# vaenyr/stable-diffusion-on-device

Measured on AMD Instinct MI355X. Metric: images/sec + per-UNet-step ms, SD v1.4 512x512 20-step PLMS, 1/2/4/8 MI355X, higher is better.
Workload: dtype f16

## Files before the change

### stable-diffusion-on-device_amd/csrc/attention.hip

```cpp
#include "common.h"
#include "sdod_hip.h"
#include "host_util.h"

#include <cstdlib>
#include <type_traits>

namespace {

struct AttnP {
    const f16* q;
    const f16* k;
    const f16* v;
    f16* out;
    int B, H, Lq, Lk;
    int ldq, ldk, ldv, ldo;
    float scale_log2;
    int causal;
};

typedef short short4v __attribute__((__vector_size__(4 * sizeof(short))));
typedef __attribute__((address_space(3))) short4v* lds_short4_ptr;

constexpr int odd16(int dv) {
    int s = (dv + 15) / 16;
    if ((s & 1) == 0) s += 1;
    return s * 16;
}

template <int D, int QT>
constexpr int attn_min_waves() { return (D == 40 || (D == 80 && QT == 1)) ? 3 : 1; }

template <int N, int I = 0, class F>
SDOD_DEVICE void static_for(F&& f) {
    if constexpr (I < N) {
        f(std::integral_constant<int, I>{});
        static_for<N, I + 1>(f);
    }
}

template <int D, int QT, bool TR, int KVS = 1>
__global__ __launch_bounds__(256 * KVS, (attn_min_waves<D, QT>())) void attn_kernel(const AttnP p) {
    constexpr int DP = ((D + 31) / 32) * 32;
    constexpr int KSTEPS = DP / 32;
    constexpr int DV = ((D + 15) / 16) * 16;
    constexpr int NDT = DV / 16;
    constexpr int KSTR = DP + 8;
    constexpr int VSTR = odd16(DV);
    constexpr int KT = 64;
    constexpr int DC = D / 8;
    constexpr int LD_IT = (KT * DC + 255) / 256;
    constexpr int STAGE = KT * (KSTR + VSTR);
    constexpr bool SUM_BY_MFMA = DV > D;
    static_assert(D % 8 == 0, "head dim must be a multiple of 8");

    extern __shared__ __attribute__((aligned(16))) char smem_raw[];
    const int grp = KVS > 1 ? (int)(threadIdx.x >> 8) : 0;
    f16* smem = reinterpret_cast<f16*>(smem_raw) + (size_t)grp * 2 * STAGE;

    const int tid = threadIdx.x & 255;
    const int lane = tid & 63;
    const int wave = tid >> 6;
    const int g = lane >> 4;
    const int li = lane & 15;
    const int nqb = (p.Lq + 64 * QT - 1) / (64 * QT);
    const int lid = xcd_remap(blockIdx.x, nqb * p.H * p.B);
    const int bh = lid / nqb;
    const int b = bh / p.H, h = bh - b * p.H;
    const int q_block = (lid - bh * nqb) * (64 * QT);

    const f16* kbase = p.k + (size_t)b * p.Lk * p.ldk + h * D;
    const f16* vbase = p.v + (size_t)b * p.Lk * p.ldv + h * D;

    {
        constexpr int KPADC = (DP - D) / 8, VPADC = (DV - D) / 8;
        for (int st = 0; st < 2; ++st) {
            f16* sK = smem + st * STAGE;
            f16* sV = sK + KT * KSTR;
            if (KPADC > 0)
                for (int idx = tid; idx < KT * KPADC; idx += 256) {
                    const int row = idx / (KPADC > 0 ? KPADC : 1), ch = idx - row * KPADC;
                    *reinterpret_cast<f16x8*>(sK + row * KSTR + D + ch * 8) = zero8();
                }
            if (VPADC > 0)
                for (int idx = tid; idx < KT * VPADC; idx += 256) {
                    const int row = idx / (VPADC > 0 ? VPADC : 1), ch = idx - row * VPADC;
                    f16x8 pad = zero8();
                    if (ch == 0) pad[0] = (f16)1.0f;
                    *reinterpret_cast<f16x8*>(sV + row * VSTR + D + ch * 8) = pad;
                }
        }
    }

    f16x8 qf[QT][KSTEPS];
    int qrow[QT];
#pragma unroll
    for (int t = 0; t < QT; ++t) {
        qrow[t] = q_block + wave * (16 * QT) + t * 16 + li;
        const f16* qp = p.q + ((size_t)b * p.Lq + qrow[t]) * p.ldq + h * D;
#pragma unroll
        for (int ks = 0; ks < KSTEPS; ++ks) {
            const int d0 = ks * 32 + g * 8;
            qf[t][ks] = (qrow[t] < p.Lq && d0 + 8 <= D) ? ldg8(qp + d0) : zero8();
        }
    }

    int kend = p.Lk;
    if (p.causal) kend = min(p.Lk, q_block + 64 * QT);
    const int NT = (kend + KT - 1) / KT;

    f16x8 rk[LD_IT], rv[LD_IT];
    const f16* kptr0[LD_IT];
    const f16* vptr0[LD_IT];
#pragma unroll
    for (int i = 0; i < LD_IT; ++i) {
        const int idx = tid + 256 * i;
        const int row = idx / DC, ch = idx - row * DC;
        kptr0[i] = kbase + (size_t)row * p.ldk + ch * 8;
        vptr0[i] = vbase + (size_t)row * p.ldv + ch * 8;
    }
    auto load_tile = [&](int t) {
        if (t * KT + KT <= p.Lk) {
            const size_t ko = (size_t)t * KT * p.ldk, vo = (size_t)t * KT * p.ldv;
#pragma unroll
            for (int i = 0; i < LD_IT; ++i) {
                if (tid + 256 * i < KT * DC) {
                    rk[i] = ldg8(kptr0[i] + ko);
                    rv[i] = ldg8(vptr0[i] + vo);
                }
            }
            return;
        }
#pragma unroll
        for (int i = 0; i < LD_IT; ++i) {
            const int idx = tid + 256 * i;
            const int row = idx / DC, ch = idx - row * DC;
            const int key = t * KT + row;
            const bool ok = (idx < KT * DC) && (key < p.Lk);
            rk[i] = ok ? ldg8(kbase + (size_t)key * p.ldk + ch * 8) : zero8();
            rv[i] = ok ? ldg8(vbase + (size_t)key * p.ldv + ch * 8) : zero8();
        }
    };
    auto store_tile = [&](int st) {
        f16* sK = smem + st * STAGE;
        f16* sV = sK + KT * KSTR;
#pragma unroll
        for (int i = 0; i < LD_IT; ++i) {
            const int idx = tid + 256 * i;
            const int row = idx / DC, ch = idx - row * DC;
            if (idx < KT * DC) {
                *reinterpret_cast<f16x8*>(sK + row * KSTR + ch * 8) = rk[i];
                *reinterpret_cast<f16x8*>(sV + row * VSTR + ch * 8) = rv[i];
            }
        }
    };

    f32x4 o[QT][NDT];
    float m_run[QT], l_run[QT];
#pragma unroll
    for (int t = 0; t < QT; ++t) {
        m_run[t] = -1e30f;
        l_run[t] = 0.f;
#pragma unroll
        for (int dt = 0; dt < NDT; ++dt) o[t][dt] = f32x4{0.f, 0.f, 0.f, 0.f};
    }

#ifdef SDOD_ATTN_ABLATE
    constexpr int abl = SDOD_ATTN_ABLATE;
#else
    constexpr int abl = 0;
#endif
    constexpr bool HOLD = D <= 80;
    auto read_vt = [&](const f16* sV, int u, int dt) -> f16x8 {
        const f16* a0 = sV + (32 * u + 4 * g + (li >> 2)) * VSTR + dt * 16 + 4 * (li & 3);
        const short4v lo = __builtin_amdgcn_ds_read_tr16_b64_v4i16((lds_short4_ptr)(a0));
        const short4v hi = __builtin_amdgcn_ds_read_tr16_b64_v4i16((lds_short4_ptr)(a0 + 16 * VSTR));
        typedef short short8v __attribute__((__vector_size__(8 * sizeof(short))));
        const short8v both = __builtin_shufflevector(lo, hi, 0, 1, 2, 3, 4, 5, 6, 7);
        return __builtin_bit_cast(f16x8, both);
    };
    auto softmax_pv = [&](auto a_c, int t, f32x4 (&s_a)[4], const f16x8 (&vfr)[HOLD ? 2 : 1][HOLD ? NDT : 1], const f16* sV) {
        constexpr int a = decltype(a_c)::value;
        const bool need_mask = (t * KT + KT > p.Lk) || (p.causal && (t * KT + KT - 1 > q_block + wave * (16 * QT)));
        if (need_mask) {
            int key0 = t * KT + g * 4;
            asm volatile("" : "+v"(key0));
#pragma unroll
            for (int c = 0; c < 4; ++c)
#pragma unroll
                for (int r = 0; r < 4; ++r) {
                    const int key = key0 + c * 16 + r;
                    const bool masked = (key >= p.Lk) | (p.causal & (key > qrow[a]));
                    s_a[c][r] = masked ? -1e30f : s_a[c][r];
                }
        }
        float mx;
        {
            const float t0 = fmaxf(fmaxf(s_a[0][0], s_a[0][1]), s_a[0][2]);
            const float t1 = fmaxf(fmaxf(s_a[0][3], s_a[1][0]), s_a[1][1]);
            const float t2 = fmaxf(fmaxf(s_a[1][2], s_a[1][3]), s_a[2][0]);
            const float t3 = fmaxf(fmaxf(s_a[2][1], s_a[2][2]), s_a[2][3]);
            const float t4 = fmaxf(fmaxf(s_a[3][0], s_a[3][1]), s_a[3][2]);
            const float u0 = fmaxf(fmaxf(t0, t1), t2);
            const float u1 = fmaxf(fmaxf(t3, t4), s_a[3][3]);
            mx = fmaxf(u0, u1);
        }
        mx = quad_rows_max(mx);
        const float m_new = fmaxf(m_run[a], mx * p.scale_log2);
        const bool rescale = __builtin_amdgcn_ballot_w64(m_new != m_run[a]) != 0;
        const float alpha = rescale ? __builtin_amdgcn_exp2f(m_run[a] - m_new) : 1.0f;
        m_run[a] = m_new;
        float rs[4] = {0.f, 0.f, 0.f, 0.f};
        const float sc = p.scale_log2, nm = -m_new;
#pragma unroll
        for (int c = 0; c < 4; ++c) {
#pragma unroll
            for (int r = 0; r < 4; ++r) {
                float v = __builtin_fmaf(s_a[c][r], sc, nm);
                if (!(abl & 2)) v = __builtin_amdgcn_exp2f(v);
                if (!SUM_BY_MFMA) rs[r] += v;
                s_a[c][r] = v;
            }
        }
        if (!SUM_BY_MFMA) l_run[a] = __builtin_fmaf(l_run[a], alpha, (rs[0] + rs[1]) + (rs[2] + rs[3]));
        if (rescale) {
#pragma unroll
            for (int dt = 0; dt < NDT; ++dt)
#pragma unroll
                for (int r = 0; r < 4; ++r) o[a][dt][r] *= alpha;
        }
        f16x8 pf[2];
#pragma unroll
        for (int u = 0; u < 2; ++u) {
            f16x8 f;
#pragma unroll
            for (int r = 0; r < 4; ++r) {
                f[r] = (f16)s_a[2 * u][r];
                f[4 + r] = (f16)s_a[2 * u + 1][r];
            }
            pf[u] = f;
        }
#pragma unroll
        for (int u = 0; u < 2; ++u) {
#pragma unroll
            for (int dt = 0; dt < NDT; ++dt) {
                f16x8 vf;
                if (TR) {
                    vf = HOLD ? vfr[u][dt] : read_vt(sV, u, dt);
                } else {
#pragma unroll
                    for (int e = 0; e < 8; ++e) vf[e] = sV[(32 * u + 16 * (e >> 2) + 4 * g + (e & 3)) * VSTR + dt * 16 + li];
                }
                o[a][dt] = mfma16(vf, pf[u], o[a][dt]);
            }
        }
    };
    auto read_k = [&](const f16* sK, f16x8 (&kf)[HOLD ? KSTEPS : 1][4]) {
        if constexpr (HOLD) {
#pragma unroll
            for (int ks = 0; ks < KSTEPS; ++ks)
#pragma unroll
                for (int c = 0; c < 4; ++c) kf[ks][c] = *reinterpret_cast<const f16x8*>(sK + (c * 16 + li) * KSTR + ks * 32 + g * 8);
        }
    };
    auto read_v = [&](const f16* sV, f16x8 (&vfr)[HOLD ? 2 : 1][HOLD ? NDT : 1]) {
        if constexpr (TR && HOLD) {
#pragma unroll
            for (int u = 0; u < 2; ++u)
#pragma unroll
                for (int dt = 0; dt < NDT; ++dt) vfr[u][dt] = read_vt(sV, u, dt);
        }
    };
    auto qk = [&](const f16* sK, const f16x8 (&kf)[HOLD ? KSTEPS : 1][4], f32x4 (&s)[QT][4]) {
#pragma unroll
        for (int a = 0; a < QT; ++a) {
#pragma unroll
            for (int c = 0; c < 4; ++c) s[a][c] = f32x4{0.f, 0.f, 0.f, 0.f};
#pragma unroll
            for (int ks = 0; ks < KSTEPS; ++ks)
#pragma unroll
                for (int c = 0; c < 4; ++c) {
                    const f16x8 k8 = HOLD ? kf[ks][c] : *reinterpret_cast<const f16x8*>(sK + (c * 16 + li) * KSTR + ks * 32 + g * 8);
                    s[a][c] = mfma16(k8, qf[a][ks], s[a][c]);
                }
        }
    };

    if (grp < NT) {
        load_tile(grp);
        store_tile(0);
    }
    __syncthreads();
    const int NTG = (NT + KVS - 1) / KVS;
    for (int it = 0; it < NTG; ++it) {
        const int t = it * KVS + grp;
        const int cur = it & 1;
        const bool has_next = t + KVS < NT;
        const f16* sK = smem + cur * STAGE;
        const f16* sV = sK + KT * KSTR;
        if (t >= NT) {
            __syncthreads();
            continue;
        }
        f16x8 kf[HOLD ? KSTEPS : 1][4];
        f16x8 vfr[HOLD ? 2 : 1][HOLD ? NDT : 1];
        read_k(sK, kf);
        read_v(sV, vfr);
        f32x4 s[QT][4];
        qk(sK, kf, s);
        if (has_next && !(abl & 1)) load_tile(t + KVS);
        static_for<QT>([&](auto a_c) { softmax_pv(a_c, t, s[decltype(a_c)::value], vfr, sV); });
        if (has_next) store_tile(cur ^ 1);
        __syncthreads();
    }

    if constexpr (KVS > 1) {
        static_assert(KVS == 2, "the merge below handles two groups");
        float* mrg = reinterpret_cast<float*>(smem_raw);
        constexpr int NV = QT * (2 + NDT * 4);
        static_assert((size_t)NV * 256 * sizeof(float) <= (size_t)KVS * 2 * STAGE * sizeof(f16), "merge buffer fits the staging LDS");
        if (grp == 1) {
#pragma unroll
            for (int a = 0; a < QT; ++a) {
                mrg[(a * (2 + NDT * 4) + 0) * 256 + tid] = m_run[a];
                mrg[(a * (2 + NDT * 4) + 1) * 256 + tid] = l_run[a];
#pragma unroll
                for (int dt = 0; dt < NDT; ++dt)
#pragma unroll
                    for (int r = 0; r < 4; ++r) mrg[(a * (2 + NDT * 4) + 2 + dt * 4 + r) * 256 + tid] = o[a][dt][r];
            }
        }
        __syncthreads();
        if (grp == 1) return;
#pragma unroll
        for (int a = 0; a < QT; ++a) {
            const float m1 = mrg[(a * (2 + NDT * 4) + 0) * 256 + tid], l1 = mrg[(a * (2 + NDT * 4) + 1) * 256 + tid];
            const float m = fmaxf(m_run[a], m1);
            const float a0 = __builtin_amdgcn_exp2f(m_run[a] - m), a1 = __builtin_amdgcn_exp2f(m1 - m);
            l_run[a] = l_run[a] * a0 + l1 * a1;
#pragma unroll
            for (int dt = 0; dt < NDT; ++dt)
#pragma unroll
                for (int r = 0; r < 4; ++r) o[a][dt][r] = o[a][dt][r] * a0 + mrg[(a * (2 + NDT * 4) + 2 + dt * 4 + r) * 256 + tid] * a1;
            m_run[a] = m;
        }
    }
#pragma unroll
    for (int a = 0; a < QT; ++a) {
        float l;
        if (SUM_BY_MFMA) {
            l = __shfl(o[a][D / 16][D % 4], ((D % 16) / 4) * 16 + li);
        } else {
            l = quad_rows_sum(l_run[a]);
        }
        const float inv = l > 0.f ? 1.0f / l : 0.f;
        if (qrow[a] < p.Lq) {
            f16* op = p.out + ((size_t)b * p.Lq + qrow[a]) * p.ldo + h * D;
#pragma unroll
            for (int dt = 0; dt < NDT; ++dt) {
                const int dv0 = dt * 16 + g * 4;
                if (dv0 < D) {
                    f16x4 hv;
#pragma unroll
                    for (int r = 0; r < 4; ++r) hv[r] = (f16)(o[a][dt][r] * inv);
                    *reinterpret_cast<f16x4*>(op + dv0) = hv;
                }
            }
        }
    }
}

template <int D, int QT, bool TR, int KVS = 1>
hipError_t attn_launch(const AttnP& p, hipStream_t st) {
    constexpr int DP = ((D + 31) / 32) * 32;
    constexpr int DV = ((D + 15) / 16) * 16;
    constexpr size_t smem = (size_t)KVS * 2 * 64 * (DP + 8 + odd16(DV)) * sizeof(f16);
    static_assert(smem <= 160 * 1024, "LDS");
    static std::atomic<unsigned long long> attr_devs{0};
    if (sdod::first_use_on_device(attr_devs)) {
        hipError_t e = hipFuncSetAttribute(reinterpret_cast<const void*>(&attn_kernel<D, QT, TR, KVS>),
                                           hipFuncAttributeMaxDynamicSharedMemorySize, (int)smem);
        if (e != hipSuccess) return e;
    }
    dim3 grid(((p.Lq + 64 * QT - 1) / (64 * QT)) * p.H * p.B);
    SDOD_LAUNCH((attn_kernel<D, QT, TR, KVS>), grid, dim3(256 * KVS), smem, st, p);
    return hipGetLastError();
}

template <int D>
hipError_t attn_dispatch(const AttnP& p, bool big, bool tr, hipStream_t st) {
    if (tr) return big ? attn_launch<D, 2, true>(p, st) : attn_launch<D, 1, true>(p, st);
    return big ? attn_launch<D, 2, false>(p, st) : attn_launch<D, 1, false>(p, st);
}

struct FoldP {
    const f16* kv; int ld_kv, k_off, v_off, L, n_img;
    const f16* wq; int ldq;
    const float* sq; const float* tq;
    const f16* wo; int ldwo;
    int heads, d, C;
    float alpha;
    f16* w1; float* s1; float* t1; f16* w2;
    int tiles_c;
    int n_w;
};
constexpr int kFoldKMax = 160;
__global__ __launch_bounds__(256) void xattn_fold_kernel(const FoldP p) {
    __shared__ __attribute__((aligned(16))) f16 sa[80][kFoldKMax + 8], sb[80][kFoldKMax + 8];
    const int tid = threadIdx.x, lane = tid & 63, wave = tid >> 6;
    const int NK = p.heads * 80, d = p.d;
    int item = blockIdx.x;
    if (item >= 2 * p.n_w) {
        const int idx = (item - 2 * p.n_w) * 256 + tid;
        if (idx >= p.n_img * NK) return;
        const int j = idx % 80, bh = idx / 80, h = bh % p.heads, img = bh / p.heads;
        if (j >= p.L) {
            p.s1[idx] = 0.f;
            p.t1[idx] = -30000.f;
            return;
        }
        const f16* kr = p.kv + ((long long)img * p.L + j) * p.ld_kv + p.k_off + h * d;
        float a = 0.f, b = 0.f;
        for (int dd = 0; dd < d; ++dd) {
            const float kval = (float)kr[dd];
            a = fmaf(kval, p.sq[h * d + dd], a);
            b = fmaf(kval, p.tq[h * d + dd], b);
        }
        p.s1[idx] = p.alpha * a;
        p.t1[idx] = p.alpha * b;
        return;
    }
    const bool second = item >= p.n_w;
    if (second) item -= p.n_w;
    const int tc = item % p.tiles_c, bh = item / p.tiles_c, h = bh % p.heads, img = bh / p.heads;
    const int KP = (d + 31) & ~31, kc = KP / 8;
    auto stage_rows = [&](f16 (*dst)[kFoldKMax + 8], const f16* base, long long row_stride, int valid_rows) {
        for (int idx = tid; idx < 80 * kc; idx += 256) {
            const int r = idx / kc, ch = idx - r * kc;
            const f16x8 v = (r < valid_rows && ch * 8 < d) ? ldg8(base + (long long)r * row_stride + ch * 8) : zero8();
            *reinterpret_cast<f16x8*>(&dst[r][ch * 8]) = v;
        }
    };
    if (!second) {
        stage_rows(sa, p.kv + (long long)img * p.L * p.ld_kv + p.k_off + h * d, p.ld_kv, p.L);
        for (int idx = tid; idx < KP * 10; idx += 256) {
            const int k = idx / 10, ch = idx - k * 10;
            const f16x8 v = k < d ? ldg8(p.wq + (long long)(h * d + k) * p.ldq + tc * 80 + ch * 8) : zero8();
#pragma unroll
            for (int e = 0; e < 8; ++e) sb[ch * 8 + e][k] = v[e];
        }
    } else {
        stage_rows(sa, p.wo + (long long)(tc * 80) * p.ldwo + h * d, p.ldwo, 80);
        stage_rows(sb, p.kv + (long long)img * p.L * p.ld_kv + p.v_off + h * d, p.ld_kv, p.L);
    }
    __syncthreads();
    const int fr = lane & 15, fg = lane >> 4;
    for (int rb = wave; rb < 5; rb += 4) {
        f32x4 acc[5];
#pragma unroll
        for (int j = 0; j < 5; ++j) acc[j] = f32x4{0.f, 0.f, 0.f, 0.f};
        for (int ks = 0; ks < KP / 32; ++ks) {
            const f16x8 fa = *reinterpret_cast<const f16x8*>(&sa[rb * 16 + fr][ks * 32 + fg * 8]);
#pragma unroll
            for (int j = 0; j < 5; ++j) {
                const f16x8 fb = *reinterpret_cast<const f16x8*>(&sb[j * 16 + fr][ks * 32 + fg * 8]);
                acc[j] = mfma16(fb, fa, acc[j]);
            }
        }
        const int m = rb * 16 + fr;
        f16* row = second ? p.w2 + ((long long)img * p.C + tc * 80 + m) * NK + h * 80
                          : p.w1 + ((long long)(img * p.heads + h) * 80 + m) * p.C + tc * 80;
        const float al = second ? 1.0f : p.alpha;
#pragma unroll
        for (int j = 0; j < 5; ++j) {
            f16x4 o;
#pragma unroll
            for (int r = 0; r < 4; ++r) o[r] = (f16)(al * acc[j][r]);
            *reinterpret_cast<f16x4*>(row + j * 16 + fg * 4) = o;
        }
    }
}

}

extern "C" int sdod_attention_f16(const void* q, const void* k, const void* v, void* out, int batch, int heads, int lq,
                                  int lk, int d, int ldq, int ldk, int ldv, int ldo, float scale, int causal,
                                  void* stream) {
    SDOD_TRY
    SDOD_REQUIRE(q && k && v && out, "null pointer");
    SDOD_REQUIRE(batch > 0 && heads > 0 && lq > 0 && lk > 0, "bad shape");
    SDOD_REQUIRE(d == 40 || d == 64 || d == 80 || d == 160, "head dim must be one of 40, 64, 80, 160");
    SDOD_REQUIRE(ldq % 8 == 0 && ldk % 8 == 0 && ldv % 8 == 0 && ldo % 4 == 0, "row strides must keep 16-byte alignment");
    SDOD_REQUIRE(ldq >= heads * d && ldk >= heads * d && ldv >= heads * d && ldo >= heads * d, "row stride < heads*d");
    SDOD_REQUIRE((((uintptr_t)q | (uintptr_t)k | (uintptr_t)v) & 15) == 0 && ((uintptr_t)out & 7) == 0, "misaligned pointer");
    AttnP p{};
    p.q = (const f16*)q; p.k = (const f16*)k; p.v = (const f16*)v; p.out = (f16*)out;
    p.B = batch; p.H = heads; p.Lq = lq; p.Lk = lk;
    p.ldq = ldq; p.ldk = ldk; p.ldv = ldv; p.ldo = ldo;
    p.scale_log2 = scale * 1.4426950408889634f;
    p.causal = causal;
    const bool no_tr = std::getenv("SDOD_ATTN_NO_TR") != nullptr;
    const bool tr = !no_tr;
    bool big = lq >= 2048 && d != 160;
    if (const char* e = std::getenv("SDOD_ATTN_QT")) big = e[0] == '2' && d != 160;
    hipStream_t st = (hipStream_t)stream;
    hipError_t e;
    switch (d) {
    case 40: e = attn_dispatch<40>(p, big, tr, st); break;
    case 64: e = attn_dispatch<64>(p, big, tr, st); break;
    case 80: {
        static const bool kvs_off = [] { const char* e2 = std::getenv("SDOD_ATTN_KVS"); return e2 && e2[0] == '0'; }();
        const long long wgs = (long long)((lq + 63) / 64) * heads * batch;
        if (!big && tr && !kvs_off && !causal && wgs <= 512 && lk >= 256) e = attn_launch<80, 1, true, 2>(p, st);
        else e = attn_dispatch<80>(p, big, tr, st);
        break;
    }
    default: e = attn_dispatch<160>(p, false, tr, st); break;
    }
    SDOD_HIP_CHECK(e);
    return 0;
    SDOD_CATCH
}

extern "C" int sdod_xattn_fold_f16(const void* kv, int ld_kv, int k_off, int v_off, int n_img, int L, const void* wq, int ldq,
                                   const void* sq, const void* tq, const void* wo, int ldwo, int heads, int d, float scale, void* w1,
                                   void* s1, void* t1, void* w2, void* stream) {
    SDOD_TRY
    SDOD_REQUIRE(kv && wq && sq && tq && wo && w1 && s1 && t1 && w2, "null pointer");
    SDOD_REQUIRE(n_img > 0 && heads > 0 && d > 0 && d <= kFoldKMax && d % 8 == 0 && L > 0 && L <= 80, "bad shape (d <= 160, d % 8 == 0, L <= 80)");
    const int C = heads * d, NK = heads * 80;
    SDOD_REQUIRE(C % 80 == 0 && ldq >= C && ldwo >= C && ld_kv >= C, "heads * d must be a multiple of 80; row strides >= heads * d");
    SDOD_REQUIRE(ld_kv % 8 == 0 && k_off % 8 == 0 && v_off % 8 == 0 && ldq % 8 == 0 && ldwo % 8 == 0 &&
                     (((uintptr_t)kv | (uintptr_t)wq | (uintptr_t)wo | (uintptr_t)w1 | (uintptr_t)w2) & 15) == 0,
                 "operands must keep 16-byte alignment");
    FoldP p{};
    p.kv = (const f16*)kv; p.ld_kv = ld_kv; p.k_off = k_off; p.v_off = v_off; p.L = L; p.n_img = n_img;
    p.wq = (const f16*)wq; p.ldq = ldq; p.sq = (const float*)sq; p.tq = (const float*)tq;
    p.wo = (const f16*)wo; p.ldwo = ldwo;
    p.heads = heads; p.d = d; p.C = C;
    p.alpha = scale * 1.4426950408889634f;
    p.w1 = (f16*)w1; p.s1 = (float*)s1; p.t1 = (float*)t1; p.w2 = (f16*)w2;
    p.tiles_c = C / 80;
    p.n_w = n_img * heads * p.tiles_c;
    const int blocks = 2 * p.n_w + (n_img * NK + 255) / 256;
    SDOD_LAUNCH(xattn_fold_kernel, dim3(blocks), dim3(256), 0, (hipStream_t)stream, p);
    SDOD_HIP_CHECK(hipGetLastError());
    return 0;
    SDOD_CATCH
}
```

Baseline: 10.47.

## Fold max subtraction into QK MFMA via padded K column and defer rescaling

For head dims with K padding (DP > D), Q is prescaled by scale*log2e and the running max is written into a padded Q lane, while the matching padded K column holds -1. The QK MFMA then emits scores already shifted by the running max. The online-softmax max and rescale of O and l are skipped unless some score exceeds a threshold (8 in log2 space), checked with an integer max and a wave ballot. This removes most per-tile fma and max-reduction work, but it quantises Q and the max to f16, which risks precision loss and overflow in exp2 up to 2^8.

```diff
diff --git a/stable-diffusion-on-device_amd/csrc/attention.hip b/stable-diffusion-on-device_amd/csrc/attention.hip
--- a/stable-diffusion-on-device_amd/csrc/attention.hip
+++ b/stable-diffusion-on-device_amd/csrc/attention.hip
@@ -2,6 +2,7 @@
 #include "sdod_hip.h"
 #include "host_util.h"
 
+#include <climits>
 #include <cstdlib>
 #include <type_traits>
 
@@ -51,6 +52,9 @@
     constexpr int LD_IT = (KT * DC + 255) / 256;
     constexpr int STAGE = KT * (KSTR + VSTR);
     constexpr bool SUM_BY_MFMA = DV > D;
+    constexpr bool DEFER = DP > D;
+    constexpr int KS_M = D / 32, G_M = (D % 32) / 8;
+    constexpr float THR = 8.0f;
     static_assert(D % 8 == 0, "head dim must be a multiple of 8");
 
     extern __shared__ __attribute__((aligned(16))) char smem_raw[];
@@ -79,7 +83,9 @@
             if (KPADC > 0)
                 for (int idx = tid; idx < KT * KPADC; idx += 256) {
                     const int row = idx / (KPADC > 0 ? KPADC : 1), ch = idx - row * KPADC;
-                    *reinterpret_cast<f16x8*>(sK + row * KSTR + D + ch * 8) = zero8();
+                    f16x8 pad = zero8();
+                    if (DEFER && ch == 0) pad[0] = (f16)-1.0f;
+                    *reinterpret_cast<f16x8*>(sK + row * KSTR + D + ch * 8) = pad;
                 }
             if (VPADC > 0)
                 for (int idx = tid; idx < KT * VPADC; idx += 256) {
@@ -101,6 +107,9 @@
         for (int ks = 0; ks < KSTEPS; ++ks) {
             const int d0 = ks * 32 + g * 8;
             qf[t][ks] = (qrow[t] < p.Lq && d0 + 8 <= D) ? ldg8(qp + d0) : zero8();
+            if (DEFER)
+#pragma unroll
+                for (int e = 0; e < 8; ++e) qf[t][ks][e] = (f16)((float)qf[t][ks][e] * p.scale_log2);
         }
     }
 
@@ -158,7 +167,7 @@
     float m_run[QT], l_run[QT];
 #pragma unroll
     for (int t = 0; t < QT; ++t) {
-        m_run[t] = -1e30f;
+        m_run[t] = DEFER ? 0.f : -1e30f;
         l_run[t] = 0.f;
 #pragma unroll
         for (int dt = 0; dt < NDT; ++dt) o[t][dt] = f32x4{0.f, 0.f, 0.f, 0.f};
@@ -178,7 +187,8 @@
         const short8v both = __builtin_shufflevector(lo, hi, 0, 1, 2, 3, 4, 5, 6, 7);
         return __builtin_bit_cast(f16x8, both);
     };
-    auto softmax_pv = [&](auto a_c, int t, f32x4 (&s_a)[4], const f16x8 (&vfr)[HOLD ? 2 : 1][HOLD ? NDT : 1], const f16* sV) {
+    auto softmax_pv = [&](auto a_c, int t, int thr, f32x4 (&s_a)[4], const f16x8 (&vfr)[HOLD ? 2 : 1][HOLD ? NDT : 1],
+                          const f16* sV) {
         constexpr int a = decltype(a_c)::value;
         const bool need_mask = (t * KT + KT > p.Lk) || (p.causal && (t * KT + KT - 1 > q_block + wave * (16 * QT)));
         if (need_mask) {
@@ -193,8 +203,7 @@
                     s_a[c][r] = masked ? -1e30f : s_a[c][r];
                 }
         }
-        float mx;
-        {
+        auto lane_max = [&]() {
             const float t0 = fmaxf(fmaxf(s_a[0][0], s_a[0][1]), s_a[0][2]);
             const float t1 = fmaxf(fmaxf(s_a[0][3], s_a[1][0]), s_a[1][1]);
             const float t2 = fmaxf(fmaxf(s_a[1][2], s_a[1][3]), s_a[2][0]);
@@ -202,31 +211,75 @@
             const float t4 = fmaxf(fmaxf(s_a[3][0], s_a[3][1]), s_a[3][2]);
             const float u0 = fmaxf(fmaxf(t0, t1), t2);
             const float u1 = fmaxf(fmaxf(t3, t4), s_a[3][3]);
-            mx = fmaxf(u0, u1);
-        }
-        mx = quad_rows_max(mx);
-        const float m_new = fmaxf(m_run[a], mx * p.scale_log2);
-        const bool rescale = __builtin_amdgcn_ballot_w64(m_new != m_run[a]) != 0;
-        const float alpha = rescale ? __builtin_amdgcn_exp2f(m_run[a] - m_new) : 1.0f;
-        m_run[a] = m_new;
+            return fmaxf(u0, u1);
+        };
         float rs[4] = {0.f, 0.f, 0.f, 0.f};
-        const float sc = p.scale_log2, nm = -m_new;
-#pragma unroll
-        for (int c = 0; c < 4; ++c) {
-#pragma unroll
-            for (int r = 0; r < 4; ++r) {
-                float v = __builtin_fmaf(s_a[c][r], sc, nm);
-                if (!(abl & 2)) v = __builtin_amdgcn_exp2f(v);
-                if (!SUM_BY_MFMA) rs[r] += v;
-                s_a[c][r] = v;
-            }
-        }
-        if (!SUM_BY_MFMA) l_run[a] = __builtin_fmaf(l_run[a], alpha, (rs[0] + rs[1]) + (rs[2] + rs[3]));
-        if (rescale) {
-#pragma unroll
-            for (int dt = 0; dt < NDT; ++dt)
-#pragma unroll
-                for (int r = 0; r < 4; ++r) o[a][dt][r] *= alpha;
+        if constexpr (DEFER) {
+            auto bi = [](float x) { return __builtin_bit_cast(int, x); };
+            auto mx3 = [](int x, int y, int z) { return max(max(x, y), z); };
+            const int t0 = mx3(bi(s_a[0][0]), bi(s_a[0][1]), bi(s_a[0][2]));
+            const int t1 = mx3(bi(s_a[0][3]), bi(s_a[1][0]), bi(s_a[1][1]));
+            const int t2 = mx3(bi(s_a[1][2]), bi(s_a[1][3]), bi(s_a[2][0]));
+            const int t3 = mx3(bi(s_a[2][1]), bi(s_a[2][2]), bi(s_a[2][3]));
+            const int t4 = mx3(bi(s_a[3][0]), bi(s_a[3][1]), bi(s_a[3][2]));
+            const int mi = max(mx3(t0, t1, t2), mx3(t3, t4, bi(s_a[3][3])));
+            if (__builtin_amdgcn_ballot_w64(mi > thr) != 0) {
+                const bool first = thr == INT_MIN;
+                const float mx = quad_rows_max(lane_max());
+                const float m_old = m_run[a];
+                float m_new = m_old;
+                if (first || mx > 0.f) m_new = (float)(f16)fminf(fmaxf(m_old + mx, -65504.f), 65504.f);
+                const float delta = m_new - m_old;
+                if (!first) {
+                    const float alpha = __builtin_amdgcn_exp2f(-delta);
+#pragma unroll
+                    for (int dt = 0; dt < NDT; ++dt)
+#pragma unroll
+                        for (int r = 0; r < 4; ++r) o[a][dt][r] *= alpha;
+                    if (!SUM_BY_MFMA) l_run[a] *= alpha;
+                }
+                m_run[a] = m_new;
+                if (g == G_M) qf[a][KS_M][0] = (f16)m_new;
+#pragma unroll
+                for (int c = 0; c < 4; ++c)
+#pragma unroll
+                    for (int r = 0; r < 4; ++r) s_a[c][r] -= delta;
+            }
+#pragma unroll
+            for (int c = 0; c < 4; ++c) {
+#pragma unroll
+                for (int r = 0; r < 4; ++r) {
+                    float v = s_a[c][r];
+                    if (!(abl & 2)) v = __builtin_amdgcn_exp2f(v);
+                    if (!SUM_BY_MFMA) rs[r] += v;
+                    s_a[c][r] = v;
+                }
+            }
+            if (!SUM_BY_MFMA) l_run[a] += (rs[0] + rs[1]) + (rs[2] + rs[3]);
+        } else {
+            const float mx = quad_rows_max(lane_max());
+            const float m_new = fmaxf(m_run[a], mx * p.scale_log2);
+            const bool rescale = __builtin_amdgcn_ballot_w64(m_new != m_run[a]) != 0;
+            const float alpha = rescale ? __builtin_amdgcn_exp2f(m_run[a] - m_new) : 1.0f;
+            m_run[a] = m_new;
+            const float sc = p.scale_log2, nm = -m_new;
+#pragma unroll
+            for (int c = 0; c < 4; ++c) {
+#pragma unroll
+                for (int r = 0; r < 4; ++r) {
+                    float v = __builtin_fmaf(s_a[c][r], sc, nm);
+                    if (!(abl & 2)) v = __builtin_amdgcn_exp2f(v);
+                    if (!SUM_BY_MFMA) rs[r] += v;
+                    s_a[c][r] = v;
+                }
+            }
+            if (!SUM_BY_MFMA) l_run[a] = __builtin_fmaf(l_run[a], alpha, (rs[0] + rs[1]) + (rs[2] + rs[3]));
+            if (rescale) {
+#pragma unroll
+                for (int dt = 0; dt < NDT; ++dt)
+#pragma unroll
+                    for (int r = 0; r < 4; ++r) o[a][dt][r] *= alpha;
+            }
         }
         f16x8 pf[2];
 #pragma unroll
@@ -291,6 +344,7 @@
     }
     __syncthreads();
     const int NTG = (NT + KVS - 1) / KVS;
+    int thr = INT_MIN;
     for (int it = 0; it < NTG; ++it) {
         const int t = it * KVS + grp;
         const int cur = it & 1;
@@ -308,7 +362,9 @@
         f32x4 s[QT][4];
         qk(sK, kf, s);
         if (has_next && !(abl & 1)) load_tile(t + KVS);
-        static_for<QT>([&](auto a_c) { softmax_pv(a_c, t, s[decltype(a_c)::value], vfr, sV); });
+        static_for<QT>([&](auto a_c) { softmax_pv(a_c, t, thr, s[decltype(a_c)::value], vfr, sV); });
+        thr = __builtin_bit_cast(int, THR);
+        asm volatile("" : "+s"(thr));
         if (has_next) store_tile(cur ^ 1);
         __syncthreads();
     }
```

Result: faster. 10.65 (median of 6 runs) (+1.7%).
